# rushi-the-neural-arch/PyTorch-DistributedTraining

Hardware: AMD Instinct MI355X
Metric: tokens/sec GPT-2-1.3B FSDP (whole node) (higher is better)
Workload: dtype bf16; 1 GPU; model=gpt2-1.3b, global_batch=96, seq_len=1024, parallelism=fsdp1, micro_batch_per_gpu=96, params=1313722368, hip_graph=False, optimizer=fused AdamW + global-norm clip

## Files before the change

### csrc/kernels/gemm.hip

```cpp
#include "common.h"
#include "gelu.h"
#include "reduce.h"
#include <stdlib.h>
#include <type_traits>

using namespace pdt;

namespace {

typedef __bf16 bf16x8_t __attribute__((ext_vector_type(8)));
typedef short v4i16 __attribute__((ext_vector_type(4)));
typedef int v4i __attribute__((ext_vector_type(4)));
typedef __attribute__((address_space(3))) v4i16 lds_v4i16;
typedef __attribute__((address_space(3))) u16x8 lds_u16x8;
typedef __attribute__((address_space(3))) void lds_void;
typedef __attribute__((address_space(3))) const char lds_cchar;

constexpr int TM = 256, TN = 256, KB = 64, NTH = 256;
constexpr int OPB = TM * KB * 2;
constexpr int STB = 2 * OPB;
constexpr int PIECES = OPB / (NTH * 16);

enum { L_NT = 0, L_TT = 1 };
enum { E_PLAIN = 0, E_BIAS = 1, E_GELU = 2, E_DGELU = 3, E_F32 = 4 };
// ... 72 lines not shown
      o1 = (uint32_t)(x * 128 + 16 * ((4 + g) ^ h));
    } else {
      const int q = (lane >> 2) & 3, p = lane & 3;
      o0 = (uint32_t)((8 * g + q) * 512 + 16 * (p >> 1) + 8 * (p & 1));
      o1 = (uint32_t)tt_f(8 * g + q);
    }
  }
  template <int S>
  __device__ __forceinline__ u16x8 read(lds_cchar* op, int blk) const {
    if (LAYOUT == L_NT) {
      return *(const lds_u16x8*)(op + blk * 16 * 128 + (S ? o1 : o0));
    } else {
      const uint32_t a = o0 + S * 32 * 512 + 16 * ((uint32_t)(2 * blk) ^ o1);
      const v4i16 x = __builtin_amdgcn_ds_read_tr16_b64_v4i16((lds_v4i16*)(op + a));
      const v4i16 y = __builtin_amdgcn_ds_read_tr16_b64_v4i16((lds_v4i16*)(op + a + 2048));
      return __builtin_bit_cast(u16x8, __builtin_shufflevector(x, y, 0, 1, 2, 3, 4, 5, 6, 7));
    }
  }
};

struct GemmArgs {
  const bf16_t* A;
  const bf16_t* B;
  void* C;
  const bf16_t* bias;
  const bf16_t* aux;
  bf16_t* aux_out;
  float* ws;
  int M, N, K;
  int64_t lda, ldb, ldc;
  int k_per_split;
  int xpr;
  int grp;
};

__device__ __forceinline__ void tile_of(const GemmArgs& p, int id, int ntiles, int& tm, int& tn) {
  const int mt = p.M / TM, nt = p.N / TN;
  const int xcd = id & 7, loc = id >> 3;
  if (p.xpr > 0) {
    const int xpc = 8 / p.xpr, rb = mt / p.xpr, cb = nt / xpc, g = p.grp, per = g * cb;
    tm = (xcd / xpc) * rb + (loc / per) * g + loc % g;
    tn = (xcd % xpc) * cb + (loc % per) / g;
  } else {
    const int q8 = ntiles >> 3, r8 = ntiles & 7;
    const int t = (xcd < r8 ? xcd * (q8 + 1) : r8 * (q8 + 1) + (xcd - r8) * q8) + loc;
    tm = t / nt;
    tn = t % nt;
  }
}

template <int LAYOUT, int EPI>
__global__ __launch_bounds__(NTH, 1) void gemm_kernel(GemmArgs p) {
  __shared__ __attribute__((aligned(16))) char smem[2 * STB];
  lds_cchar* const lds = (lds_cchar*)(lds_void*)smem;
  const uint32_t lds_addr = (uint32_t)(uintptr_t)(lds_void*)smem;
  const int tid = threadIdx.x, w = tid >> 6, lane = tid & 63;
  const int wr = w >> 1, wc = w & 1;
  const int ntiles = (int)gridDim.x;
  int tm, tn;
  tile_of(p, blockIdx.x, ntiles, tm, tn);
  const int m0 = tm * TM, n0 = tn * TN;
  const int kbeg = blockIdx.y * p.k_per_split;
  const int T = min(p.K - kbeg, p.k_per_split) / KB;

  Dma<LAYOUT> da, db;
  da.init(p.lda, w, lane);
// ... 188 lines not shown
      __syncthreads();
      p.ws[(int64_t)tm * p.N + n0 + tid] = red[tid] + red[256 + tid];
    }
  }
  }
}

}
#include "gemm_kloop.inc"
namespace {

constexpr int RING = 2 * STB;
constexpr int STAGE_BYTES = 32768;
constexpr int SMEM3 = RING + STAGE_BYTES;

template <int I, int N, class F>
__device__ __forceinline__ void sfor(F&& f) {
  if constexpr (I < N) {
    f(std::integral_constant<int, I>{});
    sfor<I + 1, N>(f);
  }
}

template <int K>
__device__ __forceinline__ f32x4 acc_tile() {
  float x, y, z, w;
  asm volatile("v_accvgpr_read_b32 %0, a%c4\n\tv_accvgpr_read_b32 %1, a%c5\n\t"
               "v_accvgpr_read_b32 %2, a%c6\n\tv_accvgpr_read_b32 %3, a%c7"
               : "=v"(x), "=v"(y), "=v"(z), "=v"(w)
               : "i"(4 * K), "i"(4 * K + 1), "i"(4 * K + 2), "i"(4 * K + 3));
  return f32x4{x, y, z, w};
}

__device__ __forceinline__ uint32_t stg_off(int q, int col) {
  return (uint32_t)(q * 512 + ((((col >> 3) ^ q) & 15) | ((col >> 3) & 16)) * 16 + (col & 7) * 2);
}
__device__ __forceinline__ int stg_row(int r, int q) { return 128 * (q >> 5) + 32 * r + (q & 31); }
__device__ __forceinline__ void stg_read(const char* img, u16x8 (&buf)[8], int w, int lane) {
#pragma unroll
  for (int it = 0; it < 8; ++it) {
    const int q = 16 * w + 2 * it + (lane >> 5), c16 = lane & 31;
    buf[it] = *reinterpret_cast<const u16x8*>(img + q * 512 + ((c16 ^ (q & 15)) & 15 | (c16 & 16)) * 16);
  }
}
typedef unsigned int u32x4 __attribute__((ext_vector_type(4)));
__device__ __forceinline__ __amdgpu_buffer_rsrc_t tile_rsrc(const bf16_t* base, int64_t ldc, int m0, int n0) {
  return __builtin_amdgcn_make_buffer_rsrc((void*)(base + (int64_t)m0 * ldc + n0), (short)0,
                                           (int)((255 * ldc + 256) * 2), 0x00020000);
}
__device__ __forceinline__ uint32_t stg_voff(int64_t ldc, int w, int lane) {
  return (uint32_t)(128 * (w >> 1) + 16 * (w & 1) + (lane >> 5)) * ((uint32_t)ldc * 2u) + (uint32_t)(lane & 31) * 16u;
}
__device__ __forceinline__ float row16_sum(float v) {
  v += __int_as_float(__builtin_amdgcn_update_dpp(0, __float_as_int(v), 0xB1, 0xF, 0xF, false));
  v += __int_as_float(__builtin_amdgcn_update_dpp(0, __float_as_int(v), 0x4E, 0xF, 0xF, false));
  v += __int_as_float(__builtin_amdgcn_update_dpp(0, __float_as_int(v), 0x141, 0xF, 0xF, false));
  v += __int_as_float(__builtin_amdgcn_update_dpp(0, __float_as_int(v), 0x140, 0xF, 0xF, false));
  return v;
}
__device__ __forceinline__ void stg_write_out(const u16x8 (&buf)[8], __amdgpu_buffer_rsrc_t rs, uint32_t vo,
                                              uint32_t ldc2, int r) {
#pragma unroll
  for (int it = 0; it < 8; ++it)
    __builtin_amdgcn_raw_buffer_store_b128(__builtin_bit_cast(u32x4, buf[it]), rs, (int)vo,
                                           (int)((32 * r + 2 * it) * ldc2), 0);
}
__device__ __forceinline__ void stg_fetch(u16x8 (&t)[8], __amdgpu_buffer_rsrc_t rs, uint32_t vo, uint32_t ldc2, int r) {
#pragma unroll
  for (int it = 0; it < 8; ++it)
    t[it] = __builtin_bit_cast(u16x8, __builtin_amdgcn_raw_buffer_load_b128(rs, (int)vo,
                                                                            (int)((32 * r + 2 * it) * ldc2), 0));
}
__device__ __forceinline__ void stg_put(char* img, const u16x8 (&t)[8], int w, int lane) {
#pragma unroll
  for (int it = 0; it < 8; ++it) {
    const int q = 16 * w + 2 * it + (lane >> 5), c16 = lane & 31;
    *reinterpret_cast<u16x8*>(img + q * 512 + ((c16 ^ (q & 15)) & 15 | (c16 & 16)) * 16) = t[it];
  }
}
__device__ __forceinline__ void stg_dma_round0(const bf16_t* src, int64_t ldc, int m0, int n0, uint32_t img_lds,
                                               int w, int lane) {
  const uint64_t base = (uint64_t)(uintptr_t)(src + (int64_t)m0 * ldc + n0);
  v4i rsrc;
  rsrc[0] = (int)(uint32_t)base;
  rsrc[1] = (int)((base >> 32) & 0xffff);
  rsrc[2] = (int)(uint32_t)((255 * ldc + 256) * 2);
  rsrc[3] = 0x00020000;
  const int hi = lane >> 5, p = lane & 31;
  const uint32_t row0 = (uint32_t)(128 * (w >> 1) + 16 * (w & 1));
  const uint32_t ldc2 = (uint32_t)ldc * 2u;
  uint32_t vo[8], so[8];
#pragma unroll
  for (int i = 0; i < 8; ++i) {
    const uint32_t c16 = (uint32_t)(((p ^ (2 * i + hi)) & 15) | (p & 16));
    vo[i] = (uint32_t)hi * ldc2 + c16 * 16u;
    so[i] = __builtin_amdgcn_readfirstlane((row0 + 2 * i) * ldc2);
  }
  const uint32_t m = __builtin_amdgcn_readfirstlane(img_lds + 16 * w * 512);
  asm volatile(
      "s_mov_b32 m0, %[m]\n\ts_nop 0\n\tbuffer_load_dwordx4 %[v0], %[rs], %[s0] offen lds\n\t"
      "s_add_u32 m0, m0, 1024\n\ts_nop 0\n\tbuffer_load_dwordx4 %[v1], %[rs], %[s1] offen lds\n\t"
      "s_add_u32 m0, m0, 1024\n\ts_nop 0\n\tbuffer_load_dwordx4 %[v2], %[rs], %[s2] offen lds\n\t"
      "s_add_u32 m0, m0, 1024\n\ts_nop 0\n\tbuffer_load_dwordx4 %[v3], %[rs], %[s3] offen lds\n\t"
      "s_add_u32 m0, m0, 1024\n\ts_nop 0\n\tbuffer_load_dwordx4 %[v4], %[rs], %[s4] offen lds\n\t"
      "s_add_u32 m0, m0, 1024\n\ts_nop 0\n\tbuffer_load_dwordx4 %[v5], %[rs], %[s5] offen lds\n\t"
      "s_add_u32 m0, m0, 1024\n\ts_nop 0\n\tbuffer_load_dwordx4 %[v6], %[rs], %[s6] offen lds\n\t"
      "s_add_u32 m0, m0, 1024\n\ts_nop 0\n\tbuffer_load_dwordx4 %[v7], %[rs], %[s7] offen lds"
      :
      : [m] "s"(m), [rs] "s"(rsrc), [v0] "v"(vo[0]), [v1] "v"(vo[1]), [v2] "v"(vo[2]), [v3] "v"(vo[3]),
        [v4] "v"(vo[4]), [v5] "v"(vo[5]), [v6] "v"(vo[6]), [v7] "v"(vo[7]), [s0] "s"(so[0]), [s1] "s"(so[1]),
        [s2] "s"(so[2]), [s3] "s"(so[3]), [s4] "s"(so[4]), [s5] "s"(so[5]), [s6] "s"(so[6]), [s7] "s"(so[7])
      : "memory", "scc");
}

__device__ __forceinline__ int item_tid(int wv) {
  int l;
  asm volatile("v_mbcnt_lo_u32_b32 %0, -1, 0\n\tv_mbcnt_hi_u32_b32 %0, -1, %0" : "=v"(l));
  return wv * 64 + l;
}
__device__ __forceinline__ int opaque_s(int x) {
  asm volatile("" : "+s"(x));
  return x;
}

__device__ __forceinline__ v4i scalar_rsrc(const void* base, uint32_t nbytes) {
  const uint64_t a = (uint64_t)(uintptr_t)base;
  v4i r;
  r[0] = (int)(uint32_t)a; r[1] = (int)((a >> 32) & 0xffff); r[2] = (int)nbytes; r[3] = 0x00020000;
  return r;
}
__device__ __forceinline__ void preload_bias(u16x4 (&b)[8], const bf16_t* bias, int n0, int lcol) {
  const v4i rs = scalar_rsrc(bias + n0, 512);
  const uint32_t vo = (uint32_t)lcol * 2u;
  asm volatile("buffer_load_dwordx2 %0, %8, %9, 0 offen offset:0\n\t"
               "buffer_load_dwordx2 %1, %8, %9, 0 offen offset:32\n\t"
               "buffer_load_dwordx2 %2, %8, %9, 0 offen offset:64\n\t"
               "buffer_load_dwordx2 %3, %8, %9, 0 offen offset:96\n\t"
               "buffer_load_dwordx2 %4, %8, %9, 0 offen offset:128\n\t"
               "buffer_load_dwordx2 %5, %8, %9, 0 offen offset:160\n\t"
               "buffer_load_dwordx2 %6, %8, %9, 0 offen offset:192\n\t"
               "buffer_load_dwordx2 %7, %8, %9, 0 offen offset:224"
               : "=&v"(b[0]), "=&v"(b[1]), "=&v"(b[2]), "=&v"(b[3]), "=&v"(b[4]), "=&v"(b[5]), "=&v"(b[6]),
                 "=&v"(b[7])
               : "v"(vo), "s"(rs)
               : "memory");
}
__device__ __forceinline__ void preload_round1(u16x8 (&t)[8], const bf16_t* src, int64_t ldc, int m0, int n0,
                                               uint32_t vo) {
  const v4i rs = scalar_rsrc(src + (int64_t)m0 * ldc + n0, (uint32_t)((255 * ldc + 256) * 2));
  const uint32_t l2 = (uint32_t)ldc * 2u;
  asm volatile("buffer_load_dwordx4 %0, %8, %9, %10 offen\n\t"
               "buffer_load_dwordx4 %1, %8, %9, %11 offen\n\t"
               "buffer_load_dwordx4 %2, %8, %9, %12 offen\n\t"
               "buffer_load_dwordx4 %3, %8, %9, %13 offen\n\t"
               "buffer_load_dwordx4 %4, %8, %9, %14 offen\n\t"
               "buffer_load_dwordx4 %5, %8, %9, %15 offen\n\t"
               "buffer_load_dwordx4 %6, %8, %9, %16 offen\n\t"
               "buffer_load_dwordx4 %7, %8, %9, %17 offen"
               : "=&v"(t[0]), "=&v"(t[1]), "=&v"(t[2]), "=&v"(t[3]), "=&v"(t[4]), "=&v"(t[5]), "=&v"(t[6]),
                 "=&v"(t[7])
               : "v"(vo), "s"(rs), "s"(32 * l2), "s"(34 * l2), "s"(36 * l2), "s"(38 * l2), "s"(40 * l2),
                 "s"(42 * l2), "s"(44 * l2), "s"(46 * l2)
               : "memory");
}
template <class V, int N>
__device__ __forceinline__ void settle(V (&x)[N]) {
#pragma unroll
  for (int i = 0; i < N; ++i) asm volatile("" : "+v"(x[i]));
}

template <int LAYOUT>
struct ItemOps {
  int tm, tn, m0, n0, split, T;
  uint32_t alo, ahi, blo, bhi;
  __device__ __forceinline__ void init(const GemmArgs& p, int item, int ntiles) {
    split = item / ntiles;
    tile_of(p, item - split * ntiles, ntiles, tm, tn);
    m0 = tm * TM; n0 = tn * TN;
    const int kbeg = split * p.k_per_split;
    T = min(p.K - kbeg, p.k_per_split) / KB;
    uint64_t a0, b0;
    if (LAYOUT == L_NT) {
      a0 = (uint64_t)(uintptr_t)p.A + ((uint64_t)m0 * p.lda + kbeg) * 2;
      b0 = (uint64_t)(uintptr_t)p.B + ((uint64_t)n0 * p.ldb + kbeg) * 2;
    } else {
      a0 = (uint64_t)(uintptr_t)p.A + ((uint64_t)kbeg * p.lda + m0) * 2;
      b0 = (uint64_t)(uintptr_t)p.B + ((uint64_t)kbeg * p.ldb + n0) * 2;
    }
    alo = (uint32_t)a0; ahi = (uint32_t)(a0 >> 32) & 0xffffu;
    blo = (uint32_t)b0; bhi = (uint32_t)(b0 >> 32) & 0xffffu;
  }
  __device__ __forceinline__ void skip2(uint64_t astep, uint64_t bstep) { skipn(2 * astep, 2 * bstep); }
  __device__ __forceinline__ void skip1(uint64_t astep, uint64_t bstep) { skipn(astep, bstep); }
  __device__ __forceinline__ void skipn(uint64_t da, uint64_t dbb) {
    const uint64_t a = (((uint64_t)ahi << 32) | alo) + da, b = (((uint64_t)bhi << 32) | blo) + dbb;
// ... 111 lines not shown
  asm volatile(MAC : PDT_STAMP_OUTS : PDT_ITEM_OPS, [voa0] "v"(voa0), [voa1] "v"(voa1), [vob0] "v"(vob0),         \
               [vob1] "v"(vob1), [rd0] "v"(rd0), [rdx] "v"(rd1)                                                  \
               : PDT_KLOOP_CLOBBERS, "s92", "s93", "s94", "s95", "s96", "s97", "s98", "s99")

  ItemOps<LAYOUT> cur;
  int item = blockIdx.x;
  cur.init(p, item, ntiles);
  int first = 1;
  while (true) {
    const int next_item = item + (int)gridDim.x;
    const bool has_next = next_item < nall;
    ItemOps<LAYOUT> nxt = cur;
    if (has_next) {
      GemmArgs q = p;
      q.M = opaque_s(p.M); q.N = opaque_s(p.N); q.xpr = opaque_s(p.xpr); q.grp = opaque_s(p.grp);
      q.K = opaque_s(p.K); q.k_per_split = opaque_s(p.k_per_split);
      nxt.init(q, next_item, opaque_s(ntiles));
    }
    const int hnx = P3 ? 0 : __builtin_amdgcn_readfirstlane((((nall - 1 - next_item) >> 31) + 1) & ~cur.T & 1);
    const int cnt = __builtin_amdgcn_readfirstlane(cur.T);
    first = __builtin_amdgcn_readfirstlane(first);
    ItemOps<LAYOUT> lo = cur;
    if (!first) lo.skip2(astep, bstep);
    lo.alo = __builtin_amdgcn_readfirstlane(lo.alo); lo.ahi = __builtin_amdgcn_readfirstlane(lo.ahi);
    lo.blo = __builtin_amdgcn_readfirstlane(lo.blo); lo.bhi = __builtin_amdgcn_readfirstlane(lo.bhi);
    uint64_t st0 = 0, st1 = 0, rt0 = 0;
    if (DIAG) { st0 = stamp(); rt0 = __builtin_amdgcn_s_memrealtime(); }
    const int ltid = item_tid(wv);
    uint32_t voa0, voa1, vob0, vob1, rd0, rd1;
    lane_ops(ltid, voa0, voa1, vob0, vob1, rd0, rd1);
    u16x4 pb[8];
    u16x8 pa[8];
    if constexpr (EPI == E_DGELU) {
      stg_dma_round0(p.aux, p.ldc, cur.m0, cur.n0, lds_addr + RING, ltid >> 6, ltid & 63);
      preload_round1(pa, p.aux, p.ldc, cur.m0, cur.n0, stg_voff(p.ldc, ltid >> 6, ltid & 63));
    }
    if constexpr (EPI == E_BIAS || EPI == E_GELU) preload_bias(pb, p.bias, cur.n0, 128 * ((ltid >> 6) & 1) + 4 * ((ltid & 63) >> 4));
    uint32_t ph[8] = {0, 0, 0, 0, 0, 0, 0, 0};
    if constexpr (DIAG) {
      if constexpr (LAYOUT == L_NT) PDT_KLOOP_NT_ASM_ST(PDT_GEMM_KLOOP_NT_STAMPS);
      else PDT_KLOOP_TT_ASM_ST(PDT_GEMM_KLOOP_TT_STAMPS);
    } else if constexpr (P3) {
      if constexpr (LAYOUT == L_NT) PDT_KLOOP_NT_ASM3(PDT_GEMM_KLOOP_NT3);
      else PDT_KLOOP_TT_ASM3(PDT_GEMM_KLOOP_TT3);
    } else {
      if constexpr (LAYOUT == L_NT) PDT_KLOOP_NT_ASM(PDT_GEMM_KLOOP_NT);
      else PDT_KLOOP_TT_ASM(PDT_GEMM_KLOOP_TT);
    }
    if constexpr (EPI == E_DGELU) settle(pa);
    if constexpr (EPI == E_BIAS || EPI == E_GELU) settle(pb);
    if (DIAG) st1 = stamp();
    const int m0 = cur.m0, n0 = cur.n0, tm = cur.tm;

    const int etid = item_tid(wv);
    {
    const int tid = etid, w = etid >> 6, lane = etid & 63, wr = w >> 1, wc = w & 1;
    const int lrow = 128 * wr + (lane & 15);
    const int lcol = 128 * wc + 4 * (lane >> 4);
    if constexpr (EPI == E_F32) {
      float* C = p.ws + (int64_t)cur.split * p.M * p.N;
      sfor<0, 64>([&](auto kc) {
        constexpr int k = decltype(kc)::value;
        const f32x4 v = acc_tile<k>();
        *reinterpret_cast<f32x4*>(C + (int64_t)(m0 + lrow + 16 * (k >> 3)) * p.N + n0 + lcol + 16 * (k & 7)) = v;
      });
    } else {
      bf16_t* C = reinterpret_cast<bf16_t*>(p.C);
      u16x8 buf[8];
      float bj[8][4];
      if constexpr (EPI == E_BIAS || EPI == E_GELU) {
#pragma unroll
        for (int j = 0; j < 8; ++j)
#pragma unroll
          for (int r = 0; r < 4; ++r) bj[j][r] = bf2f(pb[j][r]);
      }
      float cs[8][4];
#pragma unroll
      for (int j = 0; j < 8; ++j)
#pragma unroll
        for (int r = 0; r < 4; ++r) cs[j][r] = 0.f;
      u16x8 aux[2][8];
      const uint32_t svo = stg_voff(p.ldc, w, lane), ldc2 = (uint32_t)(p.ldc * 2);
      const __amdgpu_buffer_rsrc_t rsc = tile_rsrc(C, p.ldc, m0, n0);
      if constexpr (EPI == E_DGELU) {
#pragma unroll
        for (int it = 0; it < 8; ++it) aux[1][it] = pa[it];
      }
      sfor<0, 4>([&](auto rc) {
        constexpr int r = decltype(rc)::value;
        if constexpr (EPI == E_DGELU && r > 0) {
          __syncthreads();
          stg_put(img, aux[r & 1], w, lane);
          if constexpr (r < 3) stg_fetch(aux[(r + 1) & 1], tile_rsrc(p.aux, p.ldc, m0, n0), svo, ldc2, r + 1);
        }
        __syncthreads();
        u16x4 dk[16];
        u16x4 hk[8];
        sfor<0, 16>([&](auto kc) {
          constexpr int kk = decltype(kc)::value, k = 16 * r + kk, i = k >> 3, j = k & 7;
          if constexpr (EPI == E_DGELU && (kk & 7) == 0) {
            sfor<0, 8>([&](auto hc) {
              constexpr int k2 = k + decltype(hc)::value, i2 = k2 >> 3, j2 = k2 & 7;
              hk[decltype(hc)::value] = *reinterpret_cast<const u16x4*>(
                  img + stg_off(32 * wr + 16 * (i2 & 1) + (lane & 15), lcol + 16 * j2));
            });
          }
          const f32x4 v = acc_tile<k>();
          const uint32_t at = stg_off(32 * wr + 16 * (i & 1) + (lane & 15), lcol + 16 * j);
          u16x4 o;
          if constexpr (EPI == E_DGELU) {
            const u16x4 hh = hk[kk & 7];
#pragma unroll
            for (int e = 0; e < 4; ++e) {
              const bf16_t gb = f2bf(v[e] * bf2f(hh[e]));
              o[e] = gb;
              cs[j][e] += bf2f(gb);
            }
          } else if constexpr (EPI == E_GELU) {
#pragma unroll
            for (int e = 0; e < 4; e += 2) {
              gelu_f32x2 y2, d2;
              gelu_fwd_grad2(gelu_f32x2{bf2f(f2bf(v[e] + bj[j][e])), bf2f(f2bf(v[e + 1] + bj[j][e + 1]))}, y2, d2);
              o[e] = f2bf(y2[0]); o[e + 1] = f2bf(y2[1]);
              dk[kk][e] = f2bf(d2[0]); dk[kk][e + 1] = f2bf(d2[1]);
            }
          } else {
#pragma unroll
            for (int e = 0; e < 4; ++e) o[e] = f2bf(EPI == E_BIAS ? v[e] + bj[j][e] : v[e]);
          }
          *reinterpret_cast<u16x4*>(img + at) = o;
        });
        __syncthreads();
        stg_read(img, buf, w, lane);
        stg_write_out(buf, rsc, svo, ldc2, r);
        if constexpr (EPI == E_GELU) {
          __syncthreads();
          sfor<0, 16>([&](auto kc) {
            constexpr int kk = decltype(kc)::value, k = 16 * r + kk, i = k >> 3, j = k & 7;
            const uint32_t at = stg_off(32 * wr + 16 * (i & 1) + (lane & 15), lcol + 16 * j);
            *reinterpret_cast<u16x4*>(img + at) = dk[kk];
          });
          __syncthreads();
          stg_read(img, buf, w, lane);
          stg_write_out(buf, tile_rsrc(p.aux_out, p.ldc, m0, n0), svo, ldc2, r);
        }
      });
      if constexpr (EPI == E_DGELU) {
#pragma unroll
        for (int j = 0; j < 8; ++j)
#pragma unroll
          for (int e = 0; e < 4; ++e) cs[j][e] = row16_sum(cs[j][e]);
        __syncthreads();
        float* red = reinterpret_cast<float*>(img);
        if ((lane & 15) == 0) {
#pragma unroll
          for (int j = 0; j < 8; ++j)
#pragma unroll
            for (int e = 0; e < 4; ++e) red[wr * 256 + lcol + 16 * j + e] = cs[j][e];
        }
        __syncthreads();
        p.ws[(int64_t)tm * p.N + n0 + tid] = red[tid] + red[256 + tid];
      }
      __syncthreads();
    }
    }
    if (DIAG) {
      const uint64_t st2 = stamp();
      if (tid == 0) {
        uint64_t* d = reinterpret_cast<uint64_t*>(p.ws) + 8 * (int64_t)item;
        d[0] = st0; d[1] = st1; d[2] = st2; d[3] = rt0;
        for (int i = 0; i < 4; ++i) d[4 + i] = ((uint64_t)ph[2 * i + 1] << 32) | ph[2 * i];
      }
    }
    if (!has_next) break;
    item = next_item;
    first = 1 - hnx;
    cur = nxt;
  }
#undef PDT_KLOOP_CLOBBERS
#undef PDT_ITEM_OPS
#undef PDT_KLOOP_NT_ASM3
#undef PDT_KLOOP_TT_ASM3
#undef PDT_KLOOP_NT_ASM_ST
#undef PDT_KLOOP_TT_ASM_ST
#undef PDT_STAMP_OUTS
#undef PDT_KLOOP_NT_ASM
#undef PDT_KLOOP_TT_ASM
}

static int persist_grid(int nitems) {
  static const int cus = [] {
    int dev = 0, n = 0;
    if (hipGetDevice(&dev) != hipSuccess || hipDeviceGetAttribute(&n, hipDeviceAttributeMultiprocessorCount, dev) !=
                                                hipSuccess)
      n = 256;
    return n;
  }();
  int g = cus < nitems ? cus : nitems;
  return g >= 8 ? g & ~7 : g;
}

bool use_p3(int layout, const GemmArgs& a, int items, int grid) {
// ... 127 lines not shown
                           int64_t K, int64_t lda, int64_t ldb, int64_t ldc, const void* bias, const void* aux,
                           void* aux_out, void* dbias, float* ws, int splits, hipStream_t s) {
  if (!pdt_gemm_ok(layout, M, N, K, lda, ldb, splits) || ldc < N || ldc % 8) return (int)hipErrorInvalidValue;
  if (K / splits < 2 * KB) return (int)hipErrorInvalidValue;
  if (epi < 0 || epi > E_DGELU) return (int)hipErrorInvalidValue;
  if (splits > 1 && (epi != E_PLAIN || !ws)) return (int)hipErrorInvalidValue;
  if ((epi == E_BIAS || epi == E_GELU) && !bias) return (int)hipErrorInvalidValue;
  if (epi == E_GELU && !aux_out) return (int)hipErrorInvalidValue;
  if (epi == E_DGELU && (!aux || !ws || !dbias)) return (int)hipErrorInvalidValue;
  GemmArgs a{};
  a.A = (const bf16_t*)A; a.B = (const bf16_t*)B; a.C = C;
  a.bias = (const bf16_t*)bias; a.aux = (const bf16_t*)aux; a.aux_out = (bf16_t*)aux_out; a.ws = ws;
  a.M = (int)M; a.N = (int)N; a.K = (int)K; a.lda = lda; a.ldb = ldb; a.ldc = ldc;
  a.k_per_split = (int)(K / splits);
  a.xpr = xcd_cut((int)(M / TM), (int)(N / TN));
  a.grp = xcd_grp((int)(M / TM), (int)(N / TN), (int)(K / splits), a.xpr);
  const int run_epi = splits > 1 ? E_F32 : epi;
  if (splits > 1) a.ldc = N;
  int err = layout == L_NT ? launch_asm_layout<L_NT>(run_epi, a, splits, s)
                           : launch_asm_layout<L_TT>(run_epi, a, splits, s);
  if (err) return err;
  if (splits > 1) {
    if (ldc != N) return (int)hipErrorInvalidValue;
    const int64_t n4 = M * N / 4;
    gemm_splitk_reduce_kernel<<<grid_for(n4, 256, 256 * 16), 256, 0, s>>>(ws, (bf16_t*)C, n4, splits, M * N);
  }
  if (epi == E_DGELU)
    red::col_reduce<bf16_t>(ws, (int)(M / TM), (int)N, (bf16_t*)dbias, ws + (M / TM) * N, 0, s);
  return (int)hipGetLastError();
}

PDT_API int pdt_gemm_stamps_epi_bf16(int layout, int epi, const void* A, const void* B, void* C, int64_t M, int64_t N,
                                     int64_t K, int64_t lda, int64_t ldb, const void* bias, void* aux_out,
                                     void* stamps, hipStream_t s);
PDT_API int pdt_gemm_stamps_bf16(int layout, const void* A, const void* B, void* C, int64_t M, int64_t N, int64_t K,
                                 int64_t lda, int64_t ldb, void* stamps, hipStream_t s) {
  if (!pdt_gemm_ok(layout, M, N, K, lda, ldb, 1) || K < 2 * KB || !stamps) return (int)hipErrorInvalidValue;
  return pdt_gemm_stamps_epi_bf16(layout, E_PLAIN, A, B, C, M, N, K, lda, ldb, nullptr, nullptr, stamps, s);
}

PDT_API int pdt_gemm_stamps_epi_bf16(int layout, int epi, const void* A, const void* B, void* C, int64_t M, int64_t N,
                                     int64_t K, int64_t lda, int64_t ldb, const void* bias, void* aux_out,
                                     void* stamps, hipStream_t s) {
  if (!pdt_gemm_ok(layout, M, N, K, lda, ldb, 1) || K < 2 * KB || !stamps) return (int)hipErrorInvalidValue;
  if (epi != E_PLAIN && (layout != L_NT || !bias || (epi == E_GELU && !aux_out) || (epi != E_BIAS && epi != E_GELU)))
    return (int)hipErrorInvalidValue;
  GemmArgs a{};
  a.A = (const bf16_t*)A; a.B = (const bf16_t*)B; a.C = C; a.ws = (float*)stamps;
  a.bias = (const bf16_t*)bias; a.aux_out = (bf16_t*)aux_out;
  a.M = (int)M; a.N = (int)N; a.K = (int)K; a.lda = lda; a.ldb = ldb; a.ldc = N; a.k_per_split = (int)K;
  a.xpr = xcd_cut((int)(M / TM), (int)(N / TN));
  a.grp = xcd_grp((int)(M / TM), (int)(N / TN), (int)K, a.xpr);
  const dim3 grid(persist_grid((int)((M / TM) * (N / TN))), 1);
  if (layout == L_TT) gemm_asm_kernel<L_TT, E_PLAIN, 1><<<grid, NTH, 0, s>>>(a);
  else if (epi == E_BIAS) gemm_asm_kernel<L_NT, E_BIAS, 1><<<grid, NTH, 0, s>>>(a);
  else if (epi == E_GELU) gemm_asm_kernel<L_NT, E_GELU, 1><<<grid, NTH, 0, s>>>(a);
  else gemm_asm_kernel<L_NT, E_PLAIN, 1><<<grid, NTH, 0, s>>>(a);
  return (int)hipGetLastError();
}
```

### pytorch_distributedtraining_amd/ops/_lib.py

```python
from __future__ import annotations

import ctypes
import os
import threading

import torch

_LIB_PATH = os.environ.get("PDT_KERNEL_LIB") or os.path.join(
    os.path.dirname(os.path.dirname(os.path.abspath(__file__))), "lib", "libpdt_kernels.so")
_lock = threading.Lock()
_lib = None
_load_error: Exception | None = None

c_void_p = ctypes.c_void_p
c_int = ctypes.c_int
c_int64 = ctypes.c_int64
c_float = ctypes.c_float

_SIGS = {
    "pdt_adamw_mt": [c_void_p, c_void_p, c_int, c_int, c_int, c_float, c_float, c_float, c_float, c_float,
                     c_float, c_float, c_int, c_void_p, c_void_p, c_void_p, c_void_p],
    "pdt_step_inc": [c_void_p, c_void_p, c_void_p],
    "pdt_lt_probe": [c_int, c_int, c_int64, c_int64, c_int64, c_int, c_int, c_int],
    "pdt_lt_matmul": [c_int, c_int, c_int64, c_int64, c_int64, c_void_p, c_void_p, c_void_p, c_void_p, c_int,
# ... 116 lines not shown
    "pdt_narrow_gemm_f32_partials": [c_int64],
    "pdt_narrow_gemm_f32": [c_void_p, c_void_p, c_void_p, c_void_p, c_int64, c_int, c_int, c_void_p, c_void_p,
                            c_int, c_int, c_void_p, c_void_p],
    "pdt_narrow_wgrad_f32_ok": [c_int64, c_int, c_int],
    "pdt_narrow_wgrad_f32": [c_void_p, c_void_p, c_void_p, c_int64, c_int, c_int, c_void_p, c_void_p],
    "pdt_narrow_wgrad_ok": [c_int64, c_int, c_int],
    "pdt_narrow_wgrad_ws_floats": [c_int64, c_int, c_int],
    "pdt_narrow_wgrad": [c_void_p, c_void_p, c_void_p, c_int64, c_int, c_int, c_int, c_void_p, c_int, c_void_p],
    "pdt_narrow_gemm_ok": [c_int64, c_int, c_int],
    "pdt_narrow_gemm_partials": [c_int64, c_int, c_int],
    "pdt_narrow_gemm": [c_void_p, c_void_p, c_void_p, c_void_p, c_int64, c_int, c_int, c_void_p, c_int, c_void_p,
                        c_int, c_int, c_int, c_int, c_void_p, c_void_p],
    "pdt_window_perm": [c_void_p, c_void_p, c_void_p, c_int64, c_int, c_int, c_int, c_int, c_int, c_int, c_void_p],
    "pdt_window_perm_f32": [c_void_p, c_void_p, c_void_p, c_int64, c_int, c_int, c_int, c_int, c_int, c_int, c_void_p],
    "pdt_im2col3x3": [c_void_p, c_int64, c_int64, c_int64, c_int64, c_int, c_int, c_int, c_int, c_int, c_void_p,
                      c_int, c_void_p],
    "pdt_pixel_shuffle_affine_fwd": [c_void_p, c_int64, c_int64, c_int64, c_int64, c_int, c_int, c_int, c_int, c_int,
                                     c_float, c_void_p, c_void_p, c_int, c_void_p],
    "pdt_pixel_shuffle_affine_bwd": [c_void_p, c_int64, c_int64, c_int64, c_int64, c_int, c_int, c_int, c_int, c_int,
                                     c_float, c_void_p, c_int, c_void_p],
    "pdt_swin_mlp_ok": [c_int, c_int],
    "pdt_swin_mlp_ws_floats": [c_int],
    "pdt_swin_mlp_bwd_blocks": [c_int64],
    "pdt_swin_mlp_fwd": [c_void_p, c_void_p, c_void_p, c_void_p, c_void_p, c_void_p, c_void_p, c_int64, c_int, c_int,
                         c_void_p],
    "pdt_swin_mlp_bwd": [c_void_p, c_void_p, c_void_p, c_void_p, c_void_p, c_void_p, c_void_p, c_void_p, c_void_p,
                         c_void_p, c_int, c_void_p, c_int, c_int64, c_int, c_int, c_void_p],
    "pdt_gemm_ok": [c_int, c_int64, c_int64, c_int64, c_int64, c_int64, c_int],
    "pdt_gemm_bf16": [c_int, c_int, c_void_p, c_void_p, c_void_p, c_int64, c_int64, c_int64, c_int64, c_int64,
                      c_int64, c_void_p, c_void_p, c_void_p, c_void_p, c_void_p, c_int, c_void_p],
    "pdt_gemm_stamps_bf16": [c_int, c_void_p, c_void_p, c_void_p, c_int64, c_int64, c_int64, c_int64, c_int64,
                             c_void_p, c_void_p],
    "pdt_gemm_stamps_epi_bf16": [c_int, c_int, c_void_p, c_void_p, c_void_p, c_int64, c_int64, c_int64, c_int64,
                                 c_int64, c_void_p, c_void_p, c_void_p, c_void_p],
    "pdt_gemm2_bf16": [c_int, c_int, c_void_p, c_void_p, c_void_p, c_int64, c_int64, c_int64, c_int64, c_int64,
                       c_int64, c_void_p, c_void_p, c_void_p, c_void_p, c_void_p, c_int, c_void_p],
    "pdt_syncbn_stats": [c_void_p, c_int64, c_int, c_int64, c_int, c_void_p, c_void_p, c_void_p],
    "pdt_syncbn_finalize": [c_void_p, c_int, c_float, c_float, c_void_p, c_void_p, c_void_p, c_void_p, c_void_p],
    "pdt_syncbn_elemt": [c_void_p, c_void_p, c_void_p, c_void_p, c_void_p, c_void_p, c_int64, c_int, c_int64, c_int,
                         c_int, c_void_p],
    "pdt_syncbn_bwd_reduce": [c_void_p, c_void_p, c_void_p, c_int64, c_int, c_int64, c_int, c_void_p, c_void_p,
                              c_void_p],
    "pdt_syncbn_bwd_elemt": [c_void_p, c_void_p, c_void_p, c_void_p, c_void_p, c_void_p, c_void_p, c_void_p,
                             c_int64, c_int, c_int64, c_int, c_int, c_void_p],
}

_RET64 = {"pdt_swin_mlp_ws_floats", "pdt_narrow_wgrad_ws_floats", "pdt_fp8_gelu_bwd_ws_floats", "pdt_flash_attn_colsum_ws_floats"}

F32, BF16, F16, F64 = 0, 1, 2, 3


def dtype_code(dt: torch.dtype) -> int:
    if dt == torch.float32:
        return F32
    if dt == torch.bfloat16:
        return BF16
    if dt == torch.float16:
        return F16
    if dt == torch.float64:
        return F64
    raise TypeError(f"unsupported dtype for HIP kernel: {dt}")


def lib_path() -> str:
    return _LIB_PATH


# ... 57 lines not shown
```

Before: 155,100 tokens/s.

## Restructure GEMM epilogue into per-wave LDS slices with pipelined stores

Rewrites the GEMM epilogue so each wave stages its output through its own LDS slice and uses wave-level barriers in place of block-wide __syncthreads. For bias and GELU epilogues, LDS writes, readbacks and global stores are software-pipelined across units, and the GELU derivative is written in the same pass. The dGELU path fetches aux in a per-wave block order. It also adds diagnostic modes and a separate stamps pointer to the stamped launch API. This removes block-wide barriers from the epilogue in exchange for more complex swizzled addressing and more registers held in flight.

New measurement: 155,600 tokens/s, median of 6. Within noise of the previous version (+0.3%).

```diff
diff --git a/csrc/kernels/gemm.hip b/csrc/kernels/gemm.hip
--- a/csrc/kernels/gemm.hip
+++ b/csrc/kernels/gemm.hip
@@ -128,6 +128,7 @@
   int k_per_split;
   int xpr;
   int grp;
+  void* stamps;
 };
 
 __device__ __forceinline__ void tile_of(const GemmArgs& p, int id, int ntiles, int& tm, int& tn) {
@@ -382,24 +383,47 @@
   return f32x4{x, y, z, w};
 }
 
-__device__ __forceinline__ uint32_t stg_off(int q, int col) {
-  return (uint32_t)(q * 512 + ((((col >> 3) ^ q) & 15) | ((col >> 3) & 16)) * 16 + (col & 7) * 2);
-}
-__device__ __forceinline__ int stg_row(int r, int q) { return 128 * (q >> 5) + 32 * r + (q & 31); }
-__device__ __forceinline__ void stg_read(const char* img, u16x8 (&buf)[8], int w, int lane) {
-#pragma unroll
-  for (int it = 0; it < 8; ++it) {
-    const int q = 16 * w + 2 * it + (lane >> 5), c16 = lane & 31;
-    buf[it] = *reinterpret_cast<const u16x8*>(img + q * 512 + ((c16 ^ (q & 15)) & 15 | (c16 & 16)) * 16);
-  }
+constexpr int SLICE = STAGE_BYTES / 4;
+__device__ __forceinline__ void wave_sync() {
+  __builtin_amdgcn_wave_barrier();
+  asm volatile("" ::: "memory");
+}
+__device__ __forceinline__ uint32_t slc_off(int q, int col) {
+  return (uint32_t)(q * 256 + (((col >> 3) ^ q) & 15) * 16 + (col & 7) * 2);
+}
+__device__ __forceinline__ uint32_t slc_seg(int it, int lane) {
+  const int q = 4 * it + (lane >> 4);
+  return (uint32_t)(q * 256 + (((lane ^ q) & 15)) * 16);
+}
+template <int RB>
+__device__ __forceinline__ uint32_t unit_off(int qrow, int g, int jj) {
+  constexpr int NC = RB / 16;
+  return (uint32_t)(qrow * RB + (((2 * jj + (g >> 1)) ^ qrow) & (NC - 1)) * 16 + (g & 1) * 8);
+}
+template <int RB>
+__device__ __forceinline__ uint32_t unit_seg(int it, int lane) {
+  constexpr int NC = RB / 16;
+  const int q = (64 / NC) * it + lane / NC;
+  return (uint32_t)(q * RB + ((lane ^ q) & (NC - 1)) * 16);
+}
+template <int RB>
+__device__ __forceinline__ uint32_t unit_voff(int64_t ldc, int w, int lane) {
+  constexpr int NC = RB / 16;
+  return (uint32_t)(128 * (w >> 1) + lane / NC) * ((uint32_t)ldc * 2u) + (uint32_t)(w & 1) * 256u +
+         (uint32_t)(lane % NC) * 16u;
+}
+__device__ __forceinline__ void slc_read(const char* slc, u16x8 (&buf)[8], int lane) {
+#pragma unroll
+  for (int it = 0; it < 8; ++it) buf[it] = *reinterpret_cast<const u16x8*>(slc + slc_seg(it, lane));
 }
 typedef unsigned int u32x4 __attribute__((ext_vector_type(4)));
 __device__ __forceinline__ __amdgpu_buffer_rsrc_t tile_rsrc(const bf16_t* base, int64_t ldc, int m0, int n0) {
   return __builtin_amdgcn_make_buffer_rsrc((void*)(base + (int64_t)m0 * ldc + n0), (short)0,
                                            (int)((255 * ldc + 256) * 2), 0x00020000);
 }
-__device__ __forceinline__ uint32_t stg_voff(int64_t ldc, int w, int lane) {
-  return (uint32_t)(128 * (w >> 1) + 16 * (w & 1) + (lane >> 5)) * ((uint32_t)ldc * 2u) + (uint32_t)(lane & 31) * 16u;
+__device__ __forceinline__ uint32_t slc_voff(int64_t ldc, int w, int lane) {
+  return (uint32_t)(128 * (w >> 1) + (lane >> 4)) * ((uint32_t)ldc * 2u) + (uint32_t)(w & 1) * 256u +
+         (uint32_t)(lane & 15) * 16u;
 }
 __device__ __forceinline__ float row16_sum(float v) {
   v += __int_as_float(__builtin_amdgcn_update_dpp(0, __float_as_int(v), 0xB1, 0xF, 0xF, false));
@@ -408,27 +432,24 @@
   v += __int_as_float(__builtin_amdgcn_update_dpp(0, __float_as_int(v), 0x140, 0xF, 0xF, false));
   return v;
 }
-__device__ __forceinline__ void stg_write_out(const u16x8 (&buf)[8], __amdgpu_buffer_rsrc_t rs, uint32_t vo,
-                                              uint32_t ldc2, int r) {
+__device__ __forceinline__ void slc_write_out(const u16x8 (&buf)[8], __amdgpu_buffer_rsrc_t rs, uint32_t vo,
+                                              uint32_t ldc2, int b) {
 #pragma unroll
   for (int it = 0; it < 8; ++it)
     __builtin_amdgcn_raw_buffer_store_b128(__builtin_bit_cast(u32x4, buf[it]), rs, (int)vo,
-                                           (int)((32 * r + 2 * it) * ldc2), 0);
-}
-__device__ __forceinline__ void stg_fetch(u16x8 (&t)[8], __amdgpu_buffer_rsrc_t rs, uint32_t vo, uint32_t ldc2, int r) {
+                                           (int)((32 * b + 4 * it) * ldc2), 0);
+}
+__device__ __forceinline__ void slc_fetch(u16x8 (&t)[8], __amdgpu_buffer_rsrc_t rs, uint32_t vo, uint32_t ldc2, int b) {
 #pragma unroll
   for (int it = 0; it < 8; ++it)
     t[it] = __builtin_bit_cast(u16x8, __builtin_amdgcn_raw_buffer_load_b128(rs, (int)vo,
-                                                                            (int)((32 * r + 2 * it) * ldc2), 0));
-}
-__device__ __forceinline__ void stg_put(char* img, const u16x8 (&t)[8], int w, int lane) {
-#pragma unroll
-  for (int it = 0; it < 8; ++it) {
-    const int q = 16 * w + 2 * it + (lane >> 5), c16 = lane & 31;
-    *reinterpret_cast<u16x8*>(img + q * 512 + ((c16 ^ (q & 15)) & 15 | (c16 & 16)) * 16) = t[it];
-  }
-}
-__device__ __forceinline__ void stg_dma_round0(const bf16_t* src, int64_t ldc, int m0, int n0, uint32_t img_lds,
+                                                                            (int)((32 * b + 4 * it) * ldc2), 0));
+}
+__device__ __forceinline__ void slc_put(char* slc, const u16x8 (&t)[8], int lane) {
+#pragma unroll
+  for (int it = 0; it < 8; ++it) *reinterpret_cast<u16x8*>(slc + slc_seg(it, lane)) = t[it];
+}
+__device__ __forceinline__ void slc_dma_block0(const bf16_t* src, int64_t ldc, int m0, int n0, uint32_t img_lds,
                                                int w, int lane) {
   const uint64_t base = (uint64_t)(uintptr_t)(src + (int64_t)m0 * ldc + n0);
   v4i rsrc;
@@ -436,30 +457,28 @@
   rsrc[1] = (int)((base >> 32) & 0xffff);
   rsrc[2] = (int)(uint32_t)((255 * ldc + 256) * 2);
   rsrc[3] = 0x00020000;
-  const int hi = lane >> 5, p = lane & 31;
-  const uint32_t row0 = (uint32_t)(128 * (w >> 1) + 16 * (w & 1));
+  const int g = lane >> 4, p = lane & 15;
   const uint32_t ldc2 = (uint32_t)ldc * 2u;
-  uint32_t vo[8], so[8];
-#pragma unroll
-  for (int i = 0; i < 8; ++i) {
-    const uint32_t c16 = (uint32_t)(((p ^ (2 * i + hi)) & 15) | (p & 16));
-    vo[i] = (uint32_t)hi * ldc2 + c16 * 16u;
-    so[i] = __builtin_amdgcn_readfirstlane((row0 + 2 * i) * ldc2);
-  }
-  const uint32_t m = __builtin_amdgcn_readfirstlane(img_lds + 16 * w * 512);
+  const uint32_t row0 = (uint32_t)(128 * (w >> 1)), col0 = (uint32_t)(w & 1) * 256u;
+  uint32_t vo[4], so[8];
+#pragma unroll
+  for (int i = 0; i < 4; ++i) vo[i] = (uint32_t)g * ldc2 + (uint32_t)((p ^ (4 * i + g)) & 15) * 16u;
+#pragma unroll
+  for (int i = 0; i < 8; ++i) so[i] = __builtin_amdgcn_readfirstlane((row0 + 4 * i) * ldc2 + col0);
+  const uint32_t m = __builtin_amdgcn_readfirstlane(img_lds + w * SLICE);
   asm volatile(
       "s_mov_b32 m0, %[m]\n\ts_nop 0\n\tbuffer_load_dwordx4 %[v0], %[rs], %[s0] offen lds\n\t"
       "s_add_u32 m0, m0, 1024\n\ts_nop 0\n\tbuffer_load_dwordx4 %[v1], %[rs], %[s1] offen lds\n\t"
       "s_add_u32 m0, m0, 1024\n\ts_nop 0\n\tbuffer_load_dwordx4 %[v2], %[rs], %[s2] offen lds\n\t"
       "s_add_u32 m0, m0, 1024\n\ts_nop 0\n\tbuffer_load_dwordx4 %[v3], %[rs], %[s3] offen lds\n\t"
-      "s_add_u32 m0, m0, 1024\n\ts_nop 0\n\tbuffer_load_dwordx4 %[v4], %[rs], %[s4] offen lds\n\t"
-      "s_add_u32 m0, m0, 1024\n\ts_nop 0\n\tbuffer_load_dwordx4 %[v5], %[rs], %[s5] offen lds\n\t"
-      "s_add_u32 m0, m0, 1024\n\ts_nop 0\n\tbuffer_load_dwordx4 %[v6], %[rs], %[s6] offen lds\n\t"
-      "s_add_u32 m0, m0, 1024\n\ts_nop 0\n\tbuffer_load_dwordx4 %[v7], %[rs], %[s7] offen lds"
+      "s_add_u32 m0, m0, 1024\n\ts_nop 0\n\tbuffer_load_dwordx4 %[v0], %[rs], %[s4] offen lds\n\t"
+      "s_add_u32 m0, m0, 1024\n\ts_nop 0\n\tbuffer_load_dwordx4 %[v1], %[rs], %[s5] offen lds\n\t"
+      "s_add_u32 m0, m0, 1024\n\ts_nop 0\n\tbuffer_load_dwordx4 %[v2], %[rs], %[s6] offen lds\n\t"
+      "s_add_u32 m0, m0, 1024\n\ts_nop 0\n\tbuffer_load_dwordx4 %[v3], %[rs], %[s7] offen lds"
       :
       : [m] "s"(m), [rs] "s"(rsrc), [v0] "v"(vo[0]), [v1] "v"(vo[1]), [v2] "v"(vo[2]), [v3] "v"(vo[3]),
-        [v4] "v"(vo[4]), [v5] "v"(vo[5]), [v6] "v"(vo[6]), [v7] "v"(vo[7]), [s0] "s"(so[0]), [s1] "s"(so[1]),
-        [s2] "s"(so[2]), [s3] "s"(so[3]), [s4] "s"(so[4]), [s5] "s"(so[5]), [s6] "s"(so[6]), [s7] "s"(so[7])
+        [s0] "s"(so[0]), [s1] "s"(so[1]), [s2] "s"(so[2]), [s3] "s"(so[3]), [s4] "s"(so[4]), [s5] "s"(so[5]),
+        [s6] "s"(so[6]), [s7] "s"(so[7])
       : "memory", "scc");
 }
 
@@ -509,8 +528,8 @@
                "buffer_load_dwordx4 %7, %8, %9, %17 offen"
                : "=&v"(t[0]), "=&v"(t[1]), "=&v"(t[2]), "=&v"(t[3]), "=&v"(t[4]), "=&v"(t[5]), "=&v"(t[6]),
                  "=&v"(t[7])
-               : "v"(vo), "s"(rs), "s"(32 * l2), "s"(34 * l2), "s"(36 * l2), "s"(38 * l2), "s"(40 * l2),
-                 "s"(42 * l2), "s"(44 * l2), "s"(46 * l2)
+               : "v"(vo), "s"(rs), "s"(32 * l2), "s"(36 * l2), "s"(40 * l2), "s"(44 * l2), "s"(48 * l2),
+                 "s"(52 * l2), "s"(56 * l2), "s"(60 * l2)
                : "memory");
 }
 template <class V, int N>
@@ -688,8 +707,8 @@
     u16x4 pb[8];
     u16x8 pa[8];
     if constexpr (EPI == E_DGELU) {
-      stg_dma_round0(p.aux, p.ldc, cur.m0, cur.n0, lds_addr + RING, ltid >> 6, ltid & 63);
-      preload_round1(pa, p.aux, p.ldc, cur.m0, cur.n0, stg_voff(p.ldc, ltid >> 6, ltid & 63));
+      slc_dma_block0(p.aux, p.ldc, cur.m0, cur.n0, lds_addr + RING, ltid >> 6, ltid & 63);
+      preload_round1(pa, p.aux, p.ldc, cur.m0, cur.n0, slc_voff(p.ldc, ltid >> 6, ltid & 63));
     }
     if constexpr (EPI == E_BIAS || EPI == E_GELU) preload_bias(pb, p.bias, cur.n0, 128 * ((ltid >> 6) & 1) + 4 * ((ltid & 63) >> 4));
     uint32_t ph[8] = {0, 0, 0, 0, 0, 0, 0, 0};
@@ -735,72 +754,124 @@
       for (int j = 0; j < 8; ++j)
 #pragma unroll
         for (int r = 0; r < 4; ++r) cs[j][r] = 0.f;
-      u16x8 aux[2][8];
-      const uint32_t svo = stg_voff(p.ldc, w, lane), ldc2 = (uint32_t)(p.ldc * 2);
+      const uint32_t ldc2 = (uint32_t)(p.ldc * 2);
       const __amdgpu_buffer_rsrc_t rsc = tile_rsrc(C, p.ldc, m0, n0);
-      if constexpr (EPI == E_DGELU) {
-#pragma unroll
-        for (int it = 0; it < 8; ++it) aux[1][it] = pa[it];
-      }
-      sfor<0, 4>([&](auto rc) {
-        constexpr int r = decltype(rc)::value;
-        if constexpr (EPI == E_DGELU && r > 0) {
-          __syncthreads();
-          stg_put(img, aux[r & 1], w, lane);
-          if constexpr (r < 3) stg_fetch(aux[(r + 1) & 1], tile_rsrc(p.aux, p.ldc, m0, n0), svo, ldc2, r + 1);
+      char* const slc = img + SLICE * w;
+      const int qrow = lane & 15, qg = lane >> 4;
+      if constexpr (EPI != E_DGELU) {
+      constexpr int RB = EPI == E_GELU ? 128 : 256;
+      constexpr int TU = RB / 32, NU = 64 / TU;
+      constexpr int NI = RB / 64, UB = 16 * RB;
+      const uint32_t uvo = unit_voff<RB>(p.ldc, w, lane);
+      u16x8 bv[2][NI], bd[2][NI];
+      auto soff = [&](int u, int it) {
+        return RB == 256 ? (uint32_t)(16 * u + 4 * it) * ldc2 : (uint32_t)(16 * (u >> 1) + 8 * it) * ldc2 + 128u * (u & 1);
+      };
+      auto readback = [&](auto uc, auto ic) {
+        constexpr int u = decltype(uc)::value, it = decltype(ic)::value;
+        if constexpr (DIAG == 3) {
+          bv[u & 1][it] = bd[u & 1][it] = u16x8{0, 0, 0, 0, 0, 0, 0, 0};
+          return;
         }
-        __syncthreads();
-        u16x4 dk[16];
-        u16x4 hk[8];
-        sfor<0, 16>([&](auto kc) {
-          constexpr int kk = decltype(kc)::value, k = 16 * r + kk, i = k >> 3, j = k & 7;
-          if constexpr (EPI == E_DGELU && (kk & 7) == 0) {
-            sfor<0, 8>([&](auto hc) {
-              constexpr int k2 = k + decltype(hc)::value, i2 = k2 >> 3, j2 = k2 & 7;
-              hk[decltype(hc)::value] = *reinterpret_cast<const u16x4*>(
-                  img + stg_off(32 * wr + 16 * (i2 & 1) + (lane & 15), lcol + 16 * j2));
-            });
+        bv[u & 1][it] = *reinterpret_cast<const u16x8*>(slc + (u & 1) * UB + unit_seg<RB>(it, lane));
+        if constexpr (EPI == E_GELU)
+          bd[u & 1][it] = *reinterpret_cast<const u16x8*>(slc + (2 + (u & 1)) * UB + unit_seg<RB>(it, lane));
+      };
+      auto store = [&](auto uc, auto ic) {
+        constexpr int u = decltype(uc)::value, it = decltype(ic)::value;
+        if constexpr (DIAG >= 2) {
+          const u16x8 xv = bv[u & 1][it];
+          asm volatile("" :: "v"(xv));
+          if constexpr (EPI == E_GELU) {
+            const u16x8 xd = bd[u & 1][it];
+            asm volatile("" :: "v"(xd));
           }
+          return;
+        }
+        __builtin_amdgcn_raw_buffer_store_b128(__builtin_bit_cast(u32x4, bv[u & 1][it]), rsc, (int)uvo,
+                                               (int)soff(u, it), 0);
+        if constexpr (EPI == E_GELU)
+          __builtin_amdgcn_raw_buffer_store_b128(__builtin_bit_cast(u32x4, bd[u & 1][it]),
+                                                 tile_rsrc(p.aux_out, p.ldc, m0, n0), (int)uvo, (int)soff(u, it), 0);
+      };
+      sfor<0, NU>([&](auto uc) {
+        constexpr int u = decltype(uc)::value;
+        sfor<0, TU>([&](auto jc) {
+          constexpr int jj = decltype(jc)::value, k = u * TU + jj, j = k & 7;
           const f32x4 v = acc_tile<k>();
-          const uint32_t at = stg_off(32 * wr + 16 * (i & 1) + (lane & 15), lcol + 16 * j);
           u16x4 o;
-          if constexpr (EPI == E_DGELU) {
-            const u16x4 hh = hk[kk & 7];
-#pragma unroll
-            for (int e = 0; e < 4; ++e) {
-              const bf16_t gb = f2bf(v[e] * bf2f(hh[e]));
-              o[e] = gb;
-              cs[j][e] += bf2f(gb);
-            }
-          } else if constexpr (EPI == E_GELU) {
+          if constexpr (EPI == E_GELU) {
+            u16x4 d;
 #pragma unroll
             for (int e = 0; e < 4; e += 2) {
               gelu_f32x2 y2, d2;
               gelu_fwd_grad2(gelu_f32x2{bf2f(f2bf(v[e] + bj[j][e])), bf2f(f2bf(v[e + 1] + bj[j][e + 1]))}, y2, d2);
               o[e] = f2bf(y2[0]); o[e + 1] = f2bf(y2[1]);
-              dk[kk][e] = f2bf(d2[0]); dk[kk][e + 1] = f2bf(d2[1]);
+              d[e] = f2bf(d2[0]); d[e + 1] = f2bf(d2[1]);
             }
+            if constexpr (DIAG == 3) asm volatile("" :: "v"(d));
+            else *reinterpret_cast<u16x4*>(slc + (2 + (u & 1)) * UB + unit_off<RB>(qrow, qg, jj)) = d;
           } else {
 #pragma unroll
             for (int e = 0; e < 4; ++e) o[e] = f2bf(EPI == E_BIAS ? v[e] + bj[j][e] : v[e]);
           }
-          *reinterpret_cast<u16x4*>(img + at) = o;
+          if constexpr (DIAG == 3) asm volatile("" :: "v"(o));
+          else *reinterpret_cast<u16x4*>(slc + (u & 1) * UB + unit_off<RB>(qrow, qg, jj)) = o;
+          if constexpr (u >= 1 && (jj & 1) == 0) readback(std::integral_constant<int, u - 1>{}, std::integral_constant<int, jj / 2>{});
+          if constexpr (u >= 2 && (jj & 1) == 1) store(std::integral_constant<int, u - 2>{}, std::integral_constant<int, jj / 2>{});
+          wave_sync();
         });
-        __syncthreads();
-        stg_read(img, buf, w, lane);
-        stg_write_out(buf, rsc, svo, ldc2, r);
-        if constexpr (EPI == E_GELU) {
-          __syncthreads();
-          sfor<0, 16>([&](auto kc) {
-            constexpr int kk = decltype(kc)::value, k = 16 * r + kk, i = k >> 3, j = k & 7;
-            const uint32_t at = stg_off(32 * wr + 16 * (i & 1) + (lane & 15), lcol + 16 * j);
-            *reinterpret_cast<u16x4*>(img + at) = dk[kk];
-          });
-          __syncthreads();
-          stg_read(img, buf, w, lane);
-          stg_write_out(buf, tile_rsrc(p.aux_out, p.ldc, m0, n0), svo, ldc2, r);
+      });
+      sfor<0, NI>([&](auto ic) { readback(std::integral_constant<int, NU - 1>{}, ic); });
+      sfor<0, NI>([&](auto ic) { store(std::integral_constant<int, NU - 2>{}, ic); });
+      sfor<0, NI>([&](auto ic) { store(std::integral_constant<int, NU - 1>{}, ic); });
+      } else {
+      u16x8 aux[2][8];
+      const uint32_t svo = slc_voff(p.ldc, w, lane);
+      const int qcol = 4 * qg;
+#pragma unroll
+      for (int it = 0; it < 8; ++it) aux[1][it] = pa[it];
+      sfor<0, 4>([&](auto bc) {
+        constexpr int b = decltype(bc)::value;
+        u16x4 ok[16];
+        u16x4 hk[16];
+        if constexpr (b > 0) {
+          slc_put(slc, aux[b & 1], lane);
+          wave_sync();
         }
+        sfor<0, 16>([&](auto hc) {
+          constexpr int k2 = decltype(hc)::value;
+          hk[k2] = *reinterpret_cast<const u16x4*>(slc + slc_off(16 * (k2 >> 3) + qrow, qcol + 16 * (k2 & 7)));
+        });
+        wave_sync();
+        if constexpr (b > 0 && DIAG < 2) slc_write_out(buf, rsc, svo, ldc2, b - 1);
+        if constexpr (b < 2) slc_fetch(aux[b & 1], tile_rsrc(p.aux, p.ldc, m0, n0), svo, ldc2, b + 2);
+        sfor<0, 16>([&](auto kc) {
+          constexpr int kk = decltype(kc)::value, k = 16 * b + kk, j = k & 7;
+          const f32x4 v = acc_tile<k>();
+          const u16x4 hh = hk[kk];
+          u16x4 o;
+#pragma unroll
+          for (int e = 0; e < 4; ++e) {
+            const bf16_t gb = f2bf(v[e] * bf2f(hh[e]));
+            o[e] = gb;
+            cs[j][e] += bf2f(gb);
+          }
+          ok[kk] = o;
+        });
+        wave_sync();
+        sfor<0, 16>([&](auto kc) {
+          constexpr int kk = decltype(kc)::value;
+          const u16x4 o = ok[kk];
+          if constexpr (DIAG == 3) asm volatile("" :: "v"(o));
+          else *reinterpret_cast<u16x4*>(slc + slc_off(16 * (kk >> 3) + qrow, qcol + 16 * (kk & 7))) = o;
+        });
+        wave_sync();
+        if constexpr (DIAG < 3) slc_read(slc, buf, lane);
+        wave_sync();
       });
+      if constexpr (DIAG < 2) slc_write_out(buf, rsc, svo, ldc2, 3);
+      }
       if constexpr (EPI == E_DGELU) {
 #pragma unroll
         for (int j = 0; j < 8; ++j)
@@ -817,13 +888,13 @@
         __syncthreads();
         p.ws[(int64_t)tm * p.N + n0 + tid] = red[tid] + red[256 + tid];
       }
-      __syncthreads();
+      if constexpr (EPI == E_DGELU || P3) __syncthreads();
     }
     }
     if (DIAG) {
       const uint64_t st2 = stamp();
       if (tid == 0) {
-        uint64_t* d = reinterpret_cast<uint64_t*>(p.ws) + 8 * (int64_t)item;
+        uint64_t* d = reinterpret_cast<uint64_t*>(p.stamps) + 8 * (int64_t)item;
         d[0] = st0; d[1] = st1; d[2] = st2; d[3] = rt0;
         for (int i = 0; i < 4; ++i) d[4 + i] = ((uint64_t)ph[2 * i + 1] << 32) | ph[2 * i];
       }
@@ -1017,29 +1088,45 @@
 
 PDT_API int pdt_gemm_stamps_epi_bf16(int layout, int epi, const void* A, const void* B, void* C, int64_t M, int64_t N,
                                      int64_t K, int64_t lda, int64_t ldb, const void* bias, void* aux_out,
-                                     void* stamps, hipStream_t s);
+                                     const void* aux, float* ws, void* dbias, int mode, void* stamps, hipStream_t s);
 PDT_API int pdt_gemm_stamps_bf16(int layout, const void* A, const void* B, void* C, int64_t M, int64_t N, int64_t K,
                                  int64_t lda, int64_t ldb, void* stamps, hipStream_t s) {
   if (!pdt_gemm_ok(layout, M, N, K, lda, ldb, 1) || K < 2 * KB || !stamps) return (int)hipErrorInvalidValue;
-  return pdt_gemm_stamps_epi_bf16(layout, E_PLAIN, A, B, C, M, N, K, lda, ldb, nullptr, nullptr, stamps, s);
+  return pdt_gemm_stamps_epi_bf16(layout, E_PLAIN, A, B, C, M, N, K, lda, ldb, nullptr, nullptr, nullptr, nullptr,
+                                  nullptr, 1, stamps, s);
+}
+
+namespace {
+template <int MODE>
+void launch_stamped_nt(int epi, const GemmArgs& a, dim3 grid, hipStream_t s) {
+  if (epi == E_BIAS) gemm_asm_kernel<L_NT, E_BIAS, MODE><<<grid, NTH, 0, s>>>(a);
+  else if (epi == E_GELU) gemm_asm_kernel<L_NT, E_GELU, MODE><<<grid, NTH, 0, s>>>(a);
+  else if (epi == E_DGELU) gemm_asm_kernel<L_NT, E_DGELU, MODE><<<grid, NTH, 0, s>>>(a);
+  else gemm_asm_kernel<L_NT, E_PLAIN, MODE><<<grid, NTH, 0, s>>>(a);
+}
 }
 
 PDT_API int pdt_gemm_stamps_epi_bf16(int layout, int epi, const void* A, const void* B, void* C, int64_t M, int64_t N,
                                      int64_t K, int64_t lda, int64_t ldb, const void* bias, void* aux_out,
-                                     void* stamps, hipStream_t s) {
+                                     const void* aux, float* ws, void* dbias, int mode, void* stamps, hipStream_t s) {
   if (!pdt_gemm_ok(layout, M, N, K, lda, ldb, 1) || K < 2 * KB || !stamps) return (int)hipErrorInvalidValue;
-  if (epi != E_PLAIN && (layout != L_NT || !bias || (epi == E_GELU && !aux_out) || (epi != E_BIAS && epi != E_GELU)))
-    return (int)hipErrorInvalidValue;
+  if (epi < E_PLAIN || epi > E_DGELU || mode < 1 || mode > 3) return (int)hipErrorInvalidValue;
+  if (layout == L_TT && (epi != E_PLAIN || mode != 1)) return (int)hipErrorInvalidValue;
+  if ((epi == E_BIAS || epi == E_GELU) && !bias) return (int)hipErrorInvalidValue;
+  if (epi == E_GELU && !aux_out) return (int)hipErrorInvalidValue;
+  if (epi == E_DGELU && (!aux || !ws || !dbias)) return (int)hipErrorInvalidValue;
   GemmArgs a{};
-  a.A = (const bf16_t*)A; a.B = (const bf16_t*)B; a.C = C; a.ws = (float*)stamps;
-  a.bias = (const bf16_t*)bias; a.aux_out = (bf16_t*)aux_out;
+  a.A = (const bf16_t*)A; a.B = (const bf16_t*)B; a.C = C; a.ws = ws; a.stamps = stamps;
+  a.bias = (const bf16_t*)bias; a.aux_out = (bf16_t*)aux_out; a.aux = (const bf16_t*)aux;
   a.M = (int)M; a.N = (int)N; a.K = (int)K; a.lda = lda; a.ldb = ldb; a.ldc = N; a.k_per_split = (int)K;
   a.xpr = xcd_cut((int)(M / TM), (int)(N / TN));
   a.grp = xcd_grp((int)(M / TM), (int)(N / TN), (int)K, a.xpr);
   const dim3 grid(persist_grid((int)((M / TM) * (N / TN))), 1);
   if (layout == L_TT) gemm_asm_kernel<L_TT, E_PLAIN, 1><<<grid, NTH, 0, s>>>(a);
-  else if (epi == E_BIAS) gemm_asm_kernel<L_NT, E_BIAS, 1><<<grid, NTH, 0, s>>>(a);
-  else if (epi == E_GELU) gemm_asm_kernel<L_NT, E_GELU, 1><<<grid, NTH, 0, s>>>(a);
-  else gemm_asm_kernel<L_NT, E_PLAIN, 1><<<grid, NTH, 0, s>>>(a);
+  else if (mode == 1) launch_stamped_nt<1>(epi, a, grid, s);
+  else if (mode == 2) launch_stamped_nt<2>(epi, a, grid, s);
+  else launch_stamped_nt<3>(epi, a, grid, s);
+  if (epi == E_DGELU && mode == 1)
+    red::col_reduce<bf16_t>(ws, (int)(M / TM), (int)N, (bf16_t*)dbias, ws + (M / TM) * N, 0, s);
   return (int)hipGetLastError();
 }
diff --git a/pytorch_distributedtraining_amd/ops/_lib.py b/pytorch_distributedtraining_amd/ops/_lib.py
--- a/pytorch_distributedtraining_amd/ops/_lib.py
+++ b/pytorch_distributedtraining_amd/ops/_lib.py
@@ -172,7 +172,7 @@
     "pdt_gemm_stamps_bf16": [c_int, c_void_p, c_void_p, c_void_p, c_int64, c_int64, c_int64, c_int64, c_int64,
                              c_void_p, c_void_p],
     "pdt_gemm_stamps_epi_bf16": [c_int, c_int, c_void_p, c_void_p, c_void_p, c_int64, c_int64, c_int64, c_int64,
-                                 c_int64, c_void_p, c_void_p, c_void_p, c_void_p],
+                                 c_int64, c_void_p, c_void_p, c_void_p, c_void_p, c_void_p, c_int, c_void_p, c_void_p],
     "pdt_gemm2_bf16": [c_int, c_int, c_void_p, c_void_p, c_void_p, c_int64, c_int64, c_int64, c_int64, c_int64,
                        c_int64, c_void_p, c_void_p, c_void_p, c_void_p, c_void_p, c_int, c_void_p],
     "pdt_syncbn_stats": [c_void_p, c_int64, c_int, c_int64, c_int, c_void_p, c_void_p, c_void_p],
```
